# andres-quintela/manette

Hardware: AMD Instinct MI355X
Metric: env-steps/sec (ec x t_max frames per update) (higher is better)
Workload: dtype fp32

## Files before the change

### include/manette_hip.h

```cpp
#ifndef MANETTE_HIP_H
#define MANETTE_HIP_H

#include <stddef.h>
#include <stdint.h>

#ifdef __cplusplus
extern "C" {
#endif

typedef void *mt_stream_t;

enum {
  MT_OK = 0,
  MT_ERR_ARG = 1,
  MT_ERR_HIP = 2,
  MT_ERR_UNSUPPORTED = 3,
  MT_ERR_WORKSPACE = 4
};

enum { MT_ARCH_NIPS = 0, MT_ARCH_NATURE = 1, MT_ARCH_PWYX = 2, MT_ARCH_LSTM = 3, MT_ARCH_BAYESIAN = 4 };
enum { MT_ACT_RELU = 0, MT_ACT_LEAKY = 1 };
enum { MT_CLIP_IGNORE = 0, MT_CLIP_GLOBAL = 1 };

#define MT_NORM_PARTIALS 512
// ... 61 lines not shown
                            int E, int T, void *ws, size_t ws_bytes, const float *pi, const float *rep,
                            const float *v, const int32_t *a_idx, const int32_t *r_idx, const float *y,
                            const float *adv, float entropy_beta, float *grad, float *loss_terms,
                            float *norm_partials, mt_stream_t stream);

int mt_sample(const float *pi, const float *rep, int batch, int num_actions, int num_reps,
              uint64_t seed, int row0, uint64_t *counters, int32_t *a_idx, int32_t *r_idx, int32_t *pair,
              mt_stream_t stream);

enum { MT_POLICY_MULTINOMIAL = 0, MT_POLICY_EGREEDY = 1, MT_POLICY_ARGMAX = 2 };
typedef struct {
  int32_t mode;
  int32_t annealed;
  double epsilon;
  double annealing_steps;
  int64_t rows_per_call;
} mt_policy;

int mt_sample_policy(const mt_policy *policy, const float *pi, const float *rep, int batch, int num_actions,
                     int num_reps, uint64_t seed, int row0, uint64_t *counters, int32_t *a_idx, int32_t *r_idx,
                     int32_t *pair, mt_stream_t stream);
int mt_policy_draw_host(const mt_policy *policy, uint64_t seed, uint64_t global_row, uint64_t counter,
                        const float *pi, int num_actions, const float *rep, int num_reps, int32_t *a, int32_t *r);

int mt_returns(const float *rewards, const float *masks, const float *values, const float *v_boot,
               double gamma, int T, int E, float *y, float *adv, mt_stream_t stream);

int mt_loss_backward(const mt_net *net, const float *params, const uint8_t *obs, int batch,
                     void *ws, size_t ws_bytes, const float *pi, const float *rep, const float *v,
                     const int32_t *a_idx, const int32_t *r_idx, const float *y, const float *adv,
                     float entropy_beta, float *grad, float *loss_terms, mt_stream_t stream);

int mt_returns_loss_backward(const mt_net *net, const float *params, const uint8_t *obs, int T, int E, void *ws,
                             size_t ws_bytes, const float *pi, const float *rep, const float *values,
                             const int32_t *a_idx, const int32_t *r_idx, const float *rewards,
                             const float *masks, const float *v_boot, double gamma, float *y, float *adv,
                             float entropy_beta, float *grad, float *loss_terms, float *norm_partials,
                             mt_stream_t stream);
int mt_returns_loss_backward_boot(const mt_net *net, const float *params, const uint8_t *obs, int T, int E, void *ws,
                                  size_t ws_bytes, const float *pi, const float *rep, const float *values,
                                  const int32_t *a_idx, const int32_t *r_idx, const float *rewards,
                                  const float *masks, const void *boot_ws, size_t boot_ws_bytes, float *v_boot,
                                  double gamma, float *y, float *adv, float entropy_beta, float *grad,
                                  float *loss_terms, float *norm_partials, mt_stream_t stream);

int mt_grad_sumsq(const float *g, size_t n, float inv_scale, float *partials, mt_stream_t stream);
// ... 105 lines not shown
```

### manette_amd/_lib.py

```python
import ctypes as C
import os

HERE = os.path.dirname(os.path.abspath(__file__))
HIP_LIB = os.environ.get('MANETTE_HIP_LIB') or os.path.join(HERE, 'libmanette_hip.so')
HOST_LIB = os.path.join(HERE, 'libmanette_host.so')

MT_ARCH = {'NIPS': 0, 'NATURE': 1, 'PWYX': 2, 'LSTM': 3, 'BAYESIAN': 4}
MT_ACT = {'relu': 0, 'leaky_relu': 1}
MT_CLIP = {'ignore': 0, 'global': 1}
MT_NORM_PARTIALS = 512
MT_COMM_UID_BYTES = 128


class MTError(RuntimeError):
    pass


class mt_rollout_buffers(C.Structure):
    _fields_ = [(n, C.c_void_p) for n in ('states', 'values', 'idx', 'pi', 'rep', 'ws')] + \
               [('ws_bytes', C.c_size_t)] + \
               [(n, C.c_void_p) for n in ('counters', 'raw')] + [('src_rows', C.c_int32)] + \
               [(n, C.c_void_p) for n in ('pair', 'pair_host', 'meta', 'row_lut', 'col_lut', 'idx_host',
                                          'staging_host', 'meta_host', 'reward_host', 'over_host',
                                          'rm_host', 'frames_host', 'sync_host', 'train_ws')] + \
# ... 39 lines not shown
    'mt_net_create': (_I, [C.POINTER(mt_net_config), C.POINTER(_P)]),
    'mt_net_destroy': (None, [_P]),
    'mt_net_num_params': (_I, [_P, C.POINTER(_SZ)]),
    'mt_net_num_vars': (_I, [_P, C.POINTER(_I)]),
    'mt_net_var_info': (_I, [_P, _I, C.c_char_p, _I, C.POINTER(C.c_int64), C.POINTER(_I),
                             C.POINTER(_SZ), C.POINTER(_F)]),
    'mt_net_feature_dim': (_I, [_P, C.POINTER(_I)]),
    'mt_net_workspace_bytes': (_I, [_P, _I, C.POINTER(_SZ)]),
    'mt_net_workspace_region': (_I, [_P, _I, _I, _I, _I, _I, C.POINTER(_SZ), C.POINTER(_SZ)]),
    'mt_forward': (_I, [_P, _P, _P, _I, _P, _SZ, _P, _P, _P, _P]),
    'mt_lstm_frames_workspace_bytes': (_I, [_P, _I, _I, C.POINTER(_SZ)]),
    'mt_lstm_frames_forward': (_I, [_P, _P, _P, _I, _I, _I, _I, _P, _SZ, _P]),
    'mt_lstm_windows_forward': (_I, [_P, _P, _P, _I, _I, _I, _P, _SZ, _P, _P, _P, _P]),
    'mt_lstm_step_forward': (_I, [_P, _P, _P, _I, _I, _I, _P, _P, _P, _SZ, _P, _P, _P, _P]),
    'mt_lstm_frames_backward': (_I, [_P, _P, _P, _P, _I, _I, _P, _SZ, _P, _P, _P, _P, _P, _P, _P, _F, _P, _P, _P, _P]),
    'mt_forward_rows': (_I, [_P, _P, _P, _I, _P, _SZ, _P, _SZ, _I, _I, _P, _P, _P, _P]),
    'mt_forward_trunk': (_I, [_P, _P, _P, _I, _P, _SZ, _P]),
    'mt_forward_trunk_stacking': (_I, [_P, _P, _P, _P, _P, C.c_uint32, _P, _I, _P, _SZ, _P, _P]),
    'mt_forward_infer': (_I, [_P, _P, _P, _I, _P, _SZ, _P, _P, _P, _P]),
    'mt_sample': (_I, [_P, _P, _I, _I, _I, C.c_uint64, _I, _P, _P, _P, _P, _P]),
    'mt_sample_policy': (_I, [C.POINTER(mt_policy), _P, _P, _I, _I, _I, C.c_uint64, _I, _P, _P, _P, _P, _P]),
    'mt_policy_draw_host': (_I, [C.POINTER(mt_policy), C.c_uint64, C.c_uint64, C.c_uint64, _P, _I, _P, _I,
                                 C.POINTER(C.c_int32), C.POINTER(C.c_int32)]),
    'mt_rollout_set_policy': (_I, [_P, C.POINTER(mt_policy)]),
    'mt_returns': (_I, [_P, _P, _P, _P, C.c_double, _I, _I, _P, _P, _P]),
    'mt_loss_backward': (_I, [_P, _P, _P, _I, _P, _SZ, _P, _P, _P, _P, _P, _P, _P, _F, _P, _P, _P]),
    'mt_dropout_redraw': (_I, [_P, _P, _I, _P, _SZ, _P, _P, _P, _P]),
    'mt_dropout_mask_host': (_I, [C.c_uint64, C.c_uint64, C.c_uint64, _F, _P]),
    'mt_returns_loss_backward': (_I, [_P, _P, _P, _I, _I, _P, _SZ, _P, _P, _P, _P, _P, _P, _P, _P, C.c_double, _P, _P,
                                      _F, _P, _P, _P, _P]),
    'mt_returns_loss_backward_boot': (_I, [_P, _P, _P, _I, _I, _P, _SZ, _P, _P, _P, _P, _P, _P, _P, _P, _SZ, _P,
                                           C.c_double, _P, _P, _F, _P, _P, _P, _P]),
    'mt_grad_sumsq': (_I, [_P, _SZ, _F, _P, _P]),
    'mt_clip_rmsprop': (_I, [_P, _P, _P, _P, _SZ, _P, _P, _F, _F, _F, _F, _I, _F, _P, _P]),
    'mt_preprocess': (_I, [_P, _P, _P, _I, _I, _I, _P, _P, _P, _P, _P]),
    'mt_preprocess_pooled': (_I, [_P, _P, _P, _I, _I, _I, _P, _P, _P, _P, _P]),
    'mt_preprocess_resized': (_I, [_P, _P, _P, _I, _I, _P, _P, _P]),
    'mt_preprocess_frames': (_I, [_P, _P, _P, _I, _I, _P, _P, _P, _P, _P]),
    'mt_memory_push': (_I, [_P, _P, _P, _P, _I, _SZ, _P]),
    'mt_host_device_pointer': (_I, [_P, C.POINTER(_P)]),
    'mt_sum_slabs': (_I, [_P, _I, _SZ, _P, _P]),
    'mt_net_get_config': (_I, [_P, C.POINTER(mt_net_config)]),
    'mt_rollout_create': (_I, [_P, _I, _I, _P, _P, C.POINTER(mt_rollout_buffers), C.c_uint64, C.POINTER(_P)]),
    'mt_rollout_destroy': (None, [_P]),
    'mt_rollout_step': (_I, [_P, _P, _I, C.POINTER(C.c_int64), _P]),
    'mt_rollout_run': (_I, [_P, _P, C.POINTER(C.c_int64), _P]),
    'mt_rollout_stats': (_I, [_P, C.POINTER(C.c_double), _I]),
# ... 95 lines not shown
```

### manette_amd/build.py

```python
import os
import shutil
import subprocess
import sys

HERE = os.path.dirname(os.path.abspath(__file__))
CSRC = os.path.join(HERE, 'csrc')
HIP_SOURCES = ['net.hip', 'misc.hip', 'rollout.hip', 'comm.hip']
HIP_HEADERS = ['common.h', 'gemm.h', 'jobs.h', 'nips_bwd.h', 'trunk_fused.h', 'lstm.h', 'dconv.h', 'nature_bwd.h',
               'bayes.h']
HOST_SOURCES = ['runner.cpp', 'crc32c.cpp']
HIP_LIB = os.path.join(HERE, 'libmanette_hip.so')
PROBE_LIB = os.path.join(HERE, 'libmanette_hip_probe.so')
HOST_LIB = os.path.join(HERE, 'libmanette_host.so')
INCLUDE = os.path.join(os.path.dirname(HERE), 'include')


def _hipcc():
    for c in (os.environ.get('HIPCC'), '/opt/rocm/bin/hipcc', shutil.which('hipcc')):
        if c and os.path.exists(c):
            return c
    raise RuntimeError('hipcc not found')


def _stale(target, deps):
    if not os.path.exists(target):
        return True
    t = os.path.getmtime(target)
    return any(os.path.getmtime(d) > t for d in deps)


def build_hip(force=False, verbose=False, out=None, defines=()):
    target = out or HIP_LIB
# ... 60 lines not shown
```

### manette_amd/csrc/misc.hip

```cpp
#include <algorithm>
#include <atomic>
#include <cmath>

#include "common.h"

namespace mt {

static thread_local char g_err[512] = "";

void set_error(const char *fmt, ...) {
  va_list ap;
  va_start(ap, fmt);
  vsnprintf(g_err, sizeof(g_err), fmt, ap);
  va_end(ap);
}

__global__ void returns_kernel(const float *__restrict__ r, const float *__restrict__ mask,
                               const float *__restrict__ V, const float *__restrict__ VT,
                               double gamma, int T, int E, float *__restrict__ y,
                               float *__restrict__ adv) {
#pragma clang fp contract(off)
  const int e = blockIdx.x * blockDim.x + threadIdx.x;
  if (e >= E) return;
  const float g32 = __fmul_rn((float)gamma, VT[e]);
  double R = (double)r[(size_t)(T - 1) * E + e] + (double)g32 * (double)mask[(size_t)(T - 1) * E + e];
  y[(size_t)(T - 1) * E + e] = (float)R;
  adv[(size_t)(T - 1) * E + e] = (float)(R - (double)V[(size_t)(T - 1) * E + e]);
// ... 403 lines not shown
  MT_CHECK_ARG(pi && rep && counters && a_idx && r_idx, "null argument");
  MT_CHECK_ARG(batch >= 1 && num_actions >= 1 && num_reps >= 1 && row0 >= 0, "bad sizes");
  if (int rc = policy_check(policy, "mt_sample_policy")) return rc;
  hipLaunchKernelGGL(sample_kernel, dim3(cdiv(batch, 64)), dim3(64), 0, (hipStream_t)stream,
                     policy ? *policy : mt_policy{}, pi, rep, batch, num_actions, num_reps, seed, row0, counters,
                     a_idx, r_idx, pair);
  MT_LAUNCHED();
  return MT_OK;
}

extern "C" int mt_policy_draw_host(const mt_policy *policy, uint64_t seed, uint64_t global_row, uint64_t counter,
                                   const float *pi, int num_actions, const float *rep, int num_reps, int32_t *a,
                                   int32_t *r) {
  MT_CHECK_ARG(pi && rep && a && r, "null argument");
  MT_CHECK_ARG(num_actions >= 1 && num_reps >= 1, "bad sizes");
  if (int rc = policy_check(policy, "mt_policy_draw_host")) return rc;
  int ai, ri;
  policy_row(policy ? *policy : mt_policy{}, pi, num_actions, rep, num_reps, seed, global_row, counter, &ai, &ri);
  *a = ai;
  *r = ri;
  return MT_OK;
}

extern "C" int mt_graph_begin(mt_stream_t stream) {
  MT_CHECK_ARG(stream != nullptr, "graph capture needs a non-default stream");
  MT_HIP(hipStreamBeginCapture((hipStream_t)stream, hipStreamCaptureModeThreadLocal));
  return MT_OK;
}

extern "C" int mt_graph_end(mt_stream_t stream, void **graph_exec) {
  MT_CHECK_ARG(stream && graph_exec, "null argument");
  hipGraph_t g = nullptr;
  MT_HIP(hipStreamEndCapture((hipStream_t)stream, &g));
  hipGraphExec_t ex = nullptr;
  hipError_t e = hipGraphInstantiate(&ex, g, nullptr, nullptr, 0);
  (void)hipGraphDestroy(g);
  if (e != hipSuccess) {
    set_error("hipGraphInstantiate failed: %s", hipGetErrorString(e));
    return MT_ERR_HIP;
  }
  *graph_exec = (void *)ex;
  return MT_OK;
}

extern "C" int mt_graph_launch(void *graph_exec, mt_stream_t stream) {
  MT_CHECK_ARG(graph_exec, "null graph");
// ... 43 lines not shown
```

### manette_amd/csrc/nips_bwd.h

```cpp
#pragma once
#include "gemm.h"
#include "trunk_fused.h"

namespace mt {

struct NipsConvBwdJob {
  const uint8_t *X = nullptr;
  const float *act1 = nullptr, *dY2 = nullptr, *W2 = nullptr;
  float *dact1 = nullptr, *slab1 = nullptr, *slab2 = nullptr;
  int B = 0, act = 0;
  float alpha = 0.f;

  static constexpr int NT = 512;
  static constexpr int XROW = 24;
  static constexpr int XPLANE = 21 * XROW;
  static constexpr int X_BYTES = 64 * XPLANE;
  static constexpr int DS = 36;
  static constexpr int DY_FLOATS = 11 * 11 * DS;
  static constexpr int WS = 36;
  static constexpr int W2_FLOATS = 16 * 16 * WS;
  static constexpr int PS = 404;
  static constexpr int MAP_FLOATS = 16 * PS;
  static constexpr int SLAB1 = 257 * 16, SLAB2 = 257 * 32;
  static constexpr size_t LDS = X_BYTES + sizeof(float) * (DY_FLOATS + W2_FLOATS + 2 * MAP_FLOATS);
  static_assert(2 * sizeof(float) * (DY_FLOATS + MAP_FLOATS) <= LDS, "pair block stage");

  __host__ __device__ int pairs() const { return (B + 1) / 2; }
  __host__ __device__ int blocks() const { return B + pairs(); }

  struct DyAct {
    f32x4 yv[2], av[4];
  };
  __device__ __forceinline__ DyAct load_dy_act(int b) const {
    const int tid = threadIdx.x;
    const f32x4 *ys = reinterpret_cast<const f32x4 *>(dY2 + (size_t)b * 81 * 32);
    const f32x4 *as = reinterpret_cast<const f32x4 *>(act1 + (size_t)b * 400 * 16);
    DyAct d;
#pragma unroll
    for (int u = 0; u < 2; ++u) d.yv[u] = ys[min(tid + NT * u, 647)];
#pragma unroll
    for (int u = 0; u < 4; ++u) d.av[u] = as[min(tid + NT * u, 1599)];
    return d;
  }
  __device__ __forceinline__ void store_dy_act(const DyAct &d, float *dyp, float *a1t) const {
    const int tid = threadIdx.x;
    for (int i = tid; i < 121 * 8; i += NT) {
      const int p = i >> 3, Y = p / 11, Xc = p - 11 * Y;
// ... 10 lines not shown
    }
#pragma unroll
    for (int u = 0; u < 4; ++u) {
      const int i = tid + NT * u;
      if (i < 1600) {
        const int p = i >> 2, c = 4 * (i & 3);
#pragma unroll
        for (int e = 0; e < 4; ++e) a1t[(c + e) * PS + p] = d.av[u][e];
      }
    }
  }

  __device__ __forceinline__ void run(int bid, float *smem) const {
    if (bid < B)
      image_block(bid, smem);
    else
      pair_block(bid - B, smem);
  }

  __device__ __forceinline__ void image_block(int b, float *smem) const {
    float *dyp = smem;
    float *w2s = dyp + DY_FLOATS;
    float *a1t = w2s + W2_FLOATS;
    float *dat = a1t + MAP_FLOATS;
    uint8_t *xq = reinterpret_cast<uint8_t *>(dat + MAP_FLOATS);
    const int tid = threadIdx.x, lane = tid & 63, w = tid >> 6;
    const int r = lane & 15, g = lane >> 4;
    MT_PROBE_AT(3, b, 0);

    const uint4 *xs = reinterpret_cast<const uint4 *>(X + (size_t)b * 84 * 84 * 4);
    uint4 xv[4];
    {
      const int it = min(tid, 84 * 6 - 1), y = it / 6, jq = it - 6 * (it / 6);
#pragma unroll
      for (int v = 0; v < 4; ++v) xv[v] = xs[y * 21 + min(4 * jq + v, 20)];
    }
    const f32x4 *wsrc = reinterpret_cast<const f32x4 *>(W2);
    f32x4 wv[4];
#pragma unroll
    for (int u = 0; u < 4; ++u) wv[u] = wsrc[tid + NT * u];
    const DyAct da = load_dy_act(b);
    store_dy_act(da, dyp, a1t);
    if (tid < 84 * 6) {
      const int y = tid / 6, jq = tid - 6 * (tid / 6);
      uint8_t *row = xq + (y & 3) * 16 * XPLANE + (y >> 2) * XROW + 4 * jq;
#pragma unroll
      for (int p = 0; p < 4; ++p) {
        const uint32_t c0 = (&xv[0].x)[p], c1 = (&xv[1].x)[p], c2 = (&xv[2].x)[p], c3 = (&xv[3].x)[p];
// ... 28 lines not shown
#pragma unroll
        for (int t = 0; t < 4; ++t) af[t] = *reinterpret_cast<const f32x4 *>(dyp + off[t] - (a * 11 + bb) * DS + co0);
      };
      f32x4 acc[4];
#pragma unroll
      for (int t = 0; t < 4; ++t) acc[t] = f32x4{0.f, 0.f, 0.f, 0.f};
      f32x4 bf, af[4];
      frags(0, bf, af);
#pragma unroll
      for (int kc = 0; kc < 8; ++kc) {
        f32x4 bn, an[4];
        if (kc + 1 < 8) frags(kc + 1, bn, an);
#pragma unroll
        for (int s = 0; s < 4; ++s)
#pragma unroll
          for (int t = 0; t < 4; ++t)
            if (t < nt) acc[t] = __builtin_amdgcn_mfma_f32_16x16x4f32(af[t][s], bf[s], acc[t], 0, 0, 0);
        if (kc + 1 < 8) {
          bf = bn;
#pragma unroll
          for (int t = 0; t < 4; ++t) af[t] = an[t];
        }
      }
#pragma unroll
      for (int t = 0; t < 4; ++t)
#pragma unroll
        for (int i = 0; i < 4; ++i) {
          const int q = 16 * (t0 + t) + 4 * g + i;
          if (q < 100) {
            const int qy = q / 10, qx = q - 10 * qy;
            const int p = (2 * qy + py) * 20 + 2 * qx + px;
            const float v = acc[t][i] * act_bwd(a1t[r * PS + p], act, alpha);
            dat[r * PS + p] = v;
            if (dact1) dact1[((size_t)b * 400 + p) * 16 + r] = v;
          }
        }
    }
    __syncthreads();
    MT_PROBE_AT(3, b, 2);

    {
      f32x4 acc[2] = {f32x4{0.f, 0.f, 0.f, 0.f}, f32x4{0.f, 0.f, 0.f, 0.f}};
      float db = 0.f;
      const uint8_t *pl = xq + ((w & 3) * 16 + r) * XPLANE + (w >> 2) * XROW;
      auto frag = [&](int kc, f32x4 &bf, uint32_t &u0, uint32_t &u1) {
        const int p0 = 16 * kc + 4 * g, oy = p0 / 20, ox0 = p0 - 20 * oy;
        bf = *reinterpret_cast<const f32x4 *>(dat + r * PS + p0);
        const uint32_t *src = reinterpret_cast<const uint32_t *>(pl + oy * XROW + ox0);
        u0 = src[0];
        u1 = __builtin_amdgcn_alignbyte(src[1], src[0], 1);
      };
      f32x4 bf;
      uint32_t u0, u1;
      frag(0, bf, u0, u1);
#pragma unroll 5
      for (int kc = 0; kc < 25; ++kc) {
        f32x4 bn;
        uint32_t n0, n1;
        frag(min(kc + 1, 24), bn, n0, n1);
#pragma unroll
        for (int s = 0; s < 4; ++s) {
          acc[0] = __builtin_amdgcn_mfma_f32_16x16x4f32((float)((u0 >> (8 * s)) & 255u), bf[s], acc[0], 0, 0, 0);
          acc[1] = __builtin_amdgcn_mfma_f32_16x16x4f32((float)((u1 >> (8 * s)) & 255u), bf[s], acc[1], 0, 0, 0);
        }
        db += (bf[0] + bf[1]) + (bf[2] + bf[3]);
        bf = bn;
        u0 = n0;
        u1 = n1;
      }
      const float sc = 1.0f / 255.0f;
      float *o = slab1 + (size_t)b * SLAB1;
#pragma unroll
      for (int mt = 0; mt < 2; ++mt)
#pragma unroll
        for (int i = 0; i < 4; ++i) o[(16 * (2 * w + mt) + 4 * g + i) * 16 + r] = acc[mt][i] * sc;
      db += __shfl_xor(db, 16, 64);
      db += __shfl_xor(db, 32, 64);
      if (w == 0 && lane < 16) o[256 * 16 + r] = db;
    }
    MT_PROBE_AT(3, b, 4);
  }

  __device__ __forceinline__ void pair_block(int q, float *smem) const {
    const int lane = threadIdx.x & 63, w = threadIdx.x >> 6;
    const int r = lane & 15, g = lane >> 4;
    const int nimg = 2 * q + 1 < B ? 2 : 1;
    float *dyp[2] = {smem, smem + DY_FLOATS + MAP_FLOATS};
    float *a1t[2] = {smem + DY_FLOATS, smem + 2 * DY_FLOATS + MAP_FLOATS};
    MT_PROBE_AT(3, B + q, 0);
    const DyAct d0 = load_dy_act(2 * q), d1 = load_dy_act(min(2 * q + 1, B - 1));
    store_dy_act(d0, dyp[0], a1t[0]);
    if (nimg == 2) store_dy_act(d1, dyp[1], a1t[1]);
    __syncthreads();
    MT_PROBE_AT(3, B + q, 1);
    f32x4 acc[2][2];
#pragma unroll
    for (int mt = 0; mt < 2; ++mt) acc[mt][0] = acc[mt][1] = f32x4{0.f, 0.f, 0.f, 0.f};
    float db0 = 0.f, db1 = 0.f;
    const int ky = w >> 1, kx0 = 2 * (w & 1);
    for (int im = 0; im < nimg; ++im) {
      const float *dy = dyp[im], *at = a1t[im];
// ... 55 lines not shown
```

### manette_amd/csrc/trunk_fused.h

```cpp
#pragma once
#include "gemm.h"

#ifdef MT_PROBE
static __device__ unsigned long long mt_probe_buf[5 * 1024 * 8];
#define MT_PROBE_AT(k, b, p)                                                                     \
  do {                                                                                           \
    if (threadIdx.x == 0 && (b) < 1024) mt_probe_buf[((k) * 1024 + (b)) * 8 + (p)] = __builtin_amdgcn_s_memrealtime(); \
  } while (0)
#else
#define MT_PROBE_AT(k, b, p) \
  do {                       \
  } while (0)
#endif

namespace mt {

template <int C>
struct FusedNips {
  static constexpr int D = C / 4;
  static constexpr int ROWS2 = 9;
  static constexpr int ROWS1 = 4;
  static constexpr int RIN = 20;
  static constexpr int OW1 = 20, CO1 = 16, KK1 = 64 * C;
  static constexpr int OW2 = 9, CO2 = 32, KK2 = 256;
  static constexpr int A1S = 20;
  static constexpr int FEAT = OW2 * CO2;
  static constexpr int FLAT = ROWS2 * FEAT;
  static constexpr int F = 256;
  static constexpr int BPE = ROWS2;
  static constexpr int M1 = ROWS1 * OW1;
  static constexpr int MT1 = (M1 + 15) / 16;
  static constexpr int KC1 = KK1 / 16, KC2 = KK2 / 16;
  static constexpr int NW = C == 4 ? 8 : 4, NT = 64 * NW;
  static constexpr bool UNITS = C == 4;
  static constexpr int U1 = UNITS ? 2 * (MT1 - 1) + 4 : 0;
  static_assert(UNITS ? (C == 4 && KC1 == 16 && KC2 == 16 && MT1 == 5 && NW == 8)
                      : (KC1 % NW == 0 && KC2 % NW == 0), "K chunks split over the waves");
  static constexpr int IN_BYTES = RIN * 84 * C;
  static constexpr int FR_BYTES = RIN * 84 * D;
  static constexpr int RED_UNITS = (U1 > 8 ? U1 : 8) * 16 * CO1;
  static constexpr int RED_FLOATS = UNITS ? (RED_UNITS > FR_BYTES ? RED_UNITS : FR_BYTES)
                                          : NW * MT1 * 16 * CO1;
  static_assert(4 * FR_BYTES <= RED_FLOATS * 4, "staged frames alias the reduction buffer");
  static constexpr int W1P = KK1 + 4;
  static constexpr int W1T_FLOATS = UNITS ? CO1 * W1P : 0;
  static constexpr size_t LDS_BYTES = IN_BYTES + sizeof(float) * (RED_FLOATS + M1 * A1S + W1T_FLOATS);
  static constexpr int FC_BN = 16, FC_BM = 16, FC_KC = FEAT / 16;
  static constexpr int FC_SPLITS = 8;
};

template <int C, bool STACK>
__device__ __forceinline__ void nips_stage_rows(const uint8_t *__restrict__ obs, const StackSrc &st, int e, int i,
                                                uint8_t *xin, uint8_t *fr) {
  using Fz = FusedNips<C>;
  const size_t row0 = ((size_t)e * 84 + 8 * i) * 84 * C;
  if constexpr (!STACK) {
    const uint4 *src = reinterpret_cast<const uint4 *>(obs + row0);
    uint4 *dst = reinterpret_cast<uint4 *>(xin);
    for (int q = threadIdx.x; q < Fz::IN_BYTES / 16; q += Fz::NT) dst[q] = src[q];
    return;
  } else {
    __shared__ int s_p;
    const uint32_t tag = st.tag_base ? ((*st.tag_base + st.tag) & 0x1fffffffu) : st.tag;
    {
      const uint4 *src = reinterpret_cast<const uint4 *>(st.prev + row0);
      uint4 *dst = reinterpret_cast<uint4 *>(xin);
      for (int q = threadIdx.x; q < Fz::IN_BYTES / 16; q += Fz::NT) dst[q] = src[q];
    }
    int p;
    if (st.ready) {
      if (threadIdx.x == 0) s_p = wait_published(st.ready, e, tag, st.status);
      MT_PROBE_AT(0, blockIdx.x, 5);
      __syncthreads();
      p = min(max(s_p, 0), 4);
      const size_t F = (size_t)84 * 84 * Fz::D, lo = 4 * e * F, hi = lo + 4 * F;
      for (int q = threadIdx.x; q < p * (Fz::FR_BYTES / 16); q += Fz::NT) {
        const int j = q / (Fz::FR_BYTES / 16), qq = q - j * (Fz::FR_BYTES / 16);
        const size_t off = (((size_t)4 * e + j) * 84 + 8 * i) * 84 * Fz::D + 16 * (size_t)qq;
        reinterpret_cast<uint4 *>(fr + j * Fz::FR_BYTES)[qq] = ld_published16(st.frames, off, lo, hi);
      }
      __syncthreads();
    } else {
      if (threadIdx.x == 0) s_p = st.count ? st.count[e] : 0;
      if (st.count) {
        const size_t f0 = ((size_t)4 * e * 84 + 8 * i) * 84 * Fz::D;
        const uint4 *fs = reinterpret_cast<const uint4 *>(st.frames + f0);
        for (int q = threadIdx.x; q < Fz::FR_BYTES / 16; q += Fz::NT) reinterpret_cast<uint4 *>(fr)[q] = fs[q];
      }
      __syncthreads();
      p = st.count ? min(max(s_p, 1), 4) : 0;
      if (p > 1) {
        for (int q = threadIdx.x; q < (p - 1) * (Fz::FR_BYTES / 16); q += Fz::NT) {
          const int j = 1 + q / (Fz::FR_BYTES / 16), qq = q - (j - 1) * (Fz::FR_BYTES / 16);
          const size_t fj = (((size_t)4 * e + j) * 84 + 8 * i) * 84 * Fz::D;
          reinterpret_cast<uint4 *>(fr + j * Fz::FR_BYTES)[qq] = reinterpret_cast<const uint4 *>(st.frames + fj)[qq];
        }
        __syncthreads();
      }
    }
    uint32_t *xw = reinterpret_cast<uint32_t *>(xin);
    uint32_t *ow = reinterpret_cast<uint32_t *>(st.out + row0);
    const int own = (i == Fz::ROWS2 - 1 ? Fz::RIN : 8) * 84 * Fz::D;
    for (int w = threadIdx.x; w < Fz::RIN * 84 * Fz::D; w += Fz::NT) {
      uint32_t v = p < 4 ? xw[w] >> (8 * p) : 0u;
      for (int j = 0; j < p; ++j) v |= (uint32_t)fr[j * Fz::FR_BYTES + w] << (8 * (4 - p + j));
      xw[w] = v;
      if (w < own) ow[w] = v;
    }
  }
}

template <int C, int NCH>
__device__ __forceinline__ f32x4 nips_conv1_unit(const uint8_t *xin, const float *w1t, int t, int c0, int r, int g) {
  using Fz = FusedNips<C>;
  f32x4 acc0 = f32x4{0.f, 0.f, 0.f, 0.f}, acc1 = acc0;
  const float sc = 1.0f / 255.0f;
  const int m = min(t * 16 + r, Fz::M1 - 1);
  const int orow = m / Fz::OW1, ox = m - orow * Fz::OW1;
  const uint8_t *xb = xin + ((4 * orow) * 84 + 4 * ox) * C;
  uint32_t au[NCH];
  f32x4 bw[NCH];
#pragma unroll
  for (int j = 0; j < NCH; ++j) {
    const int kpos = 4 * (c0 + j) + g;
    au[j] = *reinterpret_cast<const uint32_t *>(xb + ((kpos >> 3) * 84 + (kpos & 7)) * C);
    bw[j] = *reinterpret_cast<const f32x4 *>(w1t + r * Fz::W1P + 16 * (c0 + j) + 4 * g);
  }
  __builtin_amdgcn_sched_barrier(0);
#pragma unroll
  for (int j = 0; j < NCH; ++j) {
    const uint32_t u = au[j];
    const f32x4 a = f32x4{(float)(u & 0xff) * sc, (float)((u >> 8) & 0xff) * sc, (float)((u >> 16) & 0xff) * sc,
                          (float)(u >> 24) * sc};
#pragma unroll
    for (int s = 0; s < 4; ++s) {
      if (j & 1)
        acc1 = __builtin_amdgcn_mfma_f32_16x16x4f32(a[s], bw[j][s], acc1, 0, 0, 0);
      else
        acc0 = __builtin_amdgcn_mfma_f32_16x16x4f32(a[s], bw[j][s], acc0, 0, 0, 0);
    }
  }
  return acc0 + acc1;
}

template <int C, bool STACK>
__global__ __launch_bounds__(FusedNips<C>::NT) void nips_conv_kernel(const uint8_t *__restrict__ obs, StackSrc st, int B,
                                                        const float *__restrict__ W1, const float *__restrict__ W2,
                                                        int act, float alpha, float *__restrict__ act2,
                                                        float *__restrict__ act1) {
  using Fz = FusedNips<C>;
  extern __shared__ __attribute__((aligned(16))) float smem[];
  float *red = smem;
  float *a1 = red + Fz::RED_FLOATS;
  float *w1t = a1 + Fz::M1 * Fz::A1S;
  uint8_t *xin = reinterpret_cast<uint8_t *>(w1t + Fz::W1T_FLOATS);
  uint8_t *fr = reinterpret_cast<uint8_t *>(red);

  const int nb = gridDim.x;
  const int bid = blockIdx.x;
  MT_PROBE_AT(0, bid, 0);
  const int L = (nb % 8 == 0) ? (bid % 8) * (nb / 8) + bid / 8 : bid;
  const int e = L / Fz::BPE, i = L - e * Fz::BPE;
  const int lane = threadIdx.x & 63, w = threadIdx.x >> 6;
  const int r = lane & 15, g = lane >> 4;

  constexpr int NW = Fz::NW;
  constexpr int J1 = Fz::UNITS ? 1 : Fz::KC1 / NW;
  float b1f[J1][4];
  if constexpr (Fz::UNITS) {
    constexpr int NQ = Fz::KK1 * Fz::CO1 / 4;
    f32x4 wv[(NQ + Fz::NT - 1) / Fz::NT];
#pragma unroll
    for (int u = 0; u < (NQ + Fz::NT - 1) / Fz::NT; ++u)
      wv[u] = reinterpret_cast<const f32x4 *>(W1)[min((int)threadIdx.x + Fz::NT * u, NQ - 1)];
#pragma unroll
    for (int u = 0; u < (NQ + Fz::NT - 1) / Fz::NT; ++u) {
      const int q = threadIdx.x + Fz::NT * u;
      if (q < NQ) {
        const int k = q >> 2, c4 = (q & 3) * 4;
#pragma unroll
        for (int e2 = 0; e2 < 4; ++e2) w1t[(c4 + e2) * Fz::W1P + k] = wv[u][e2];
      }
    }
  } else {
#pragma unroll
    for (int j = 0; j < J1; ++j) {
      const int k0 = 16 * (w + NW * j) + 4 * g;
#pragma unroll
      for (int s = 0; s < 4; ++s) b1f[j][s] = W1[(size_t)(k0 + s) * Fz::CO1 + r];
    }
  }
  nips_stage_rows<C, STACK>(obs, st, e, i, xin, fr);
  __syncthreads();
  MT_PROBE_AT(0, bid, 1);

  if constexpr (Fz::UNITS) {
    const int wu = __builtin_amdgcn_readfirstlane(w);
    const f32x4 acc = nips_conv1_unit<C, 8>(xin, w1t, wu >> 1, 8 * (wu & 1), r, g);
    f32x4 acc4 = f32x4{0.f, 0.f, 0.f, 0.f};
    if (wu < 4) acc4 = nips_conv1_unit<C, 4>(xin, w1t, 4, 4 * wu, r, g);
    MT_PROBE_AT(0, bid, 6);
#pragma unroll
    for (int q = 0; q < 4; ++q) red[(w * 16 + g * 4 + q) * Fz::CO1 + r] = acc[q];
    if (wu < 4)
#pragma unroll
      for (int q = 0; q < 4; ++q) red[((8 + w) * 16 + g * 4 + q) * Fz::CO1 + r] = acc4[q];
  } else   {
    f32x4 acc[Fz::MT1];
#pragma unroll
    for (int t = 0; t < Fz::MT1; ++t) acc[t] = f32x4{0.f, 0.f, 0.f, 0.f};
    const float sc = 1.0f / 255.0f;
#pragma unroll
    for (int j = 0; j < J1; ++j) {
      const int k0 = 16 * (w + NW * j) + 4 * g;
      const int kpos = k0 / C, ci = k0 - kpos * C;
      const int ky = kpos >> 3, kx = kpos & 7;
      f32x4 a[Fz::MT1];
#pragma unroll
      for (int t = 0; t < Fz::MT1; ++t) {
        const int m = min(t * 16 + r, Fz::M1 - 1);
        const int orow = m / Fz::OW1, ox = m - orow * Fz::OW1;
        const uint32_t u = *reinterpret_cast<const uint32_t *>(xin + ((4 * orow + ky) * 84 + 4 * ox + kx) * C + ci);
        a[t] = f32x4{(float)(u & 0xff) * sc, (float)((u >> 8) & 0xff) * sc, (float)((u >> 16) & 0xff) * sc,
                     (float)(u >> 24) * sc};
      }
#pragma unroll
      for (int s = 0; s < 4; ++s)
#pragma unroll
        for (int t = 0; t < Fz::MT1; ++t) acc[t] = __builtin_amdgcn_mfma_f32_16x16x4f32(a[t][s], b1f[j][s], acc[t], 0, 0, 0);
    }
    MT_PROBE_AT(0, bid, 6);
#pragma unroll
    for (int t = 0; t < Fz::MT1; ++t)
#pragma unroll
      for (int q = 0; q < 4; ++q) red[(w * Fz::MT1 * 16 + t * 16 + g * 4 + q) * Fz::CO1 + r] = acc[t][q];
  }
  constexpr int J2 = Fz::UNITS ? 4 : Fz::KC2 / NW;
  constexpr int NT2 = Fz::UNITS ? 1 : 2;
  float b2f[J2][NT2][4];
#pragma unroll
  for (int j = 0; j < J2; ++j) {
    const int k0 = 16 * (Fz::UNITS ? 4 * ((w >> 1) & 3) + j : w + NW * j) + 4 * g;
#pragma unroll
    for (int nt = 0; nt < NT2; ++nt)
#pragma unroll
      for (int s = 0; s < 4; ++s)
        b2f[j][nt][s] = W2[(size_t)(k0 + s) * Fz::CO2 + (Fz::UNITS ? (w & 1) : nt) * 16 + r];
  }
  __syncthreads();
  MT_PROBE_AT(0, bid, 7);
  {
    const float *b1 = W1 + (size_t)Fz::KK1 * Fz::CO1;
    constexpr int P = Fz::MT1 * 16 * Fz::CO1;
    for (int idx = threadIdx.x; idx < Fz::M1 * Fz::CO1; idx += Fz::NT) {
      const int m = idx / Fz::CO1, n = idx - m * Fz::CO1;
      float s;
      if constexpr (Fz::UNITS) {
        const int t = m >> 4, rr = m & 15;
        if (t < 4)
          s = red[((2 * t) * 16 + rr) * Fz::CO1 + n] + red[((2 * t + 1) * 16 + rr) * Fz::CO1 + n];
        else
          s = ((red[(8 * 16 + rr) * Fz::CO1 + n] + red[(9 * 16 + rr) * Fz::CO1 + n]) + red[(10 * 16 + rr) * Fz::CO1 + n]) +
              red[(11 * 16 + rr) * Fz::CO1 + n];
      } else {
        s = red[idx];
#pragma unroll
        for (int v = 1; v < NW; ++v) s += red[v * P + idx];
      }
      const float y = act_fwd(s + b1[n], act, alpha);
      a1[m * Fz::A1S + n] = y;
      const int orow = m / Fz::OW1, cx = m - orow * Fz::OW1;
      if (act1 && (orow < 2 || i == Fz::ROWS2 - 1))
        act1[(((size_t)e * Fz::OW1 + 2 * i + orow) * Fz::OW1 + cx) * Fz::CO1 + n] = y;
    }
  }
  __syncthreads();
  MT_PROBE_AT(0, bid, 2);

  if constexpr (Fz::UNITS) {
    if (w < 8) {
      const int kq = w >> 1;
      f32x4 acc0 = f32x4{0.f, 0.f, 0.f, 0.f}, acc1 = acc0;
      const int ox = min(r, Fz::OW2 - 1);
#pragma unroll
      for (int j = 0; j < J2; ++j) {
        const f32x4 a = *reinterpret_cast<const f32x4 *>(a1 + (kq * Fz::OW1 + 2 * ox + j) * Fz::A1S + 4 * g);
#pragma unroll
        for (int s = 0; s < 4; ++s) {
          if (j & 1)
            acc1 = __builtin_amdgcn_mfma_f32_16x16x4f32(a[s], b2f[j][0][s], acc1, 0, 0, 0);
          else
            acc0 = __builtin_amdgcn_mfma_f32_16x16x4f32(a[s], b2f[j][0][s], acc0, 0, 0, 0);
        }
      }
      const f32x4 acc = acc0 + acc1;
#pragma unroll
      for (int q = 0; q < 4; ++q) red[(w * 16 + g * 4 + q) * 16 + r] = acc[q];
    }
  } else   {
// ... 325 lines not shown
```

Measured before the change: 765,300.

## Use split-bf16 MFMA for NIPS conv1 forward and weight-gradient

Replaces the fp32 16x16x4 MFMA loops in the fused NIPS conv1 forward and in the conv1 weight-gradient backward with bf16 MFMAs. Byte inputs are exactly representable in bf16, and the fp32 operands (weights, dact) are split into three bf16 parts (hi/mid/lo) so the result stays close to fp32. The forward path also drops the cross-wave LDS reduction and an extra barrier, because each wave now covers the full K for one tile and applies bias and activation directly. In exchange it runs three MFMAs per operand pair, uses more LDS for the bf16 staging buffers, and gives slightly different rounding.

```diff
diff --git a/include/manette_hip.h b/include/manette_hip.h
--- a/include/manette_hip.h
+++ b/include/manette_hip.h
@@ -107,6 +107,8 @@
                      int32_t *pair, mt_stream_t stream);
 int mt_policy_draw_host(const mt_policy *policy, uint64_t seed, uint64_t global_row, uint64_t counter,
                         const float *pi, int num_actions, const float *rep, int num_reps, int32_t *a, int32_t *r);
+
+int mt_split3_bf16_host(const float *x, size_t n, uint16_t *parts, uint16_t *bytes);
 
 int mt_returns(const float *rewards, const float *masks, const float *values, const float *v_boot,
                double gamma, int T, int E, float *y, float *adv, mt_stream_t stream);
diff --git a/manette_amd/_lib.py b/manette_amd/_lib.py
--- a/manette_amd/_lib.py
+++ b/manette_amd/_lib.py
@@ -85,7 +85,8 @@
     'mt_sample_policy': (_I, [C.POINTER(mt_policy), _P, _P, _I, _I, _I, C.c_uint64, _I, _P, _P, _P, _P, _P]),
     'mt_policy_draw_host': (_I, [C.POINTER(mt_policy), C.c_uint64, C.c_uint64, C.c_uint64, _P, _I, _P, _I,
                                  C.POINTER(C.c_int32), C.POINTER(C.c_int32)]),
-    'mt_rollout_set_policy': (_I, [_P, C.POINTER(mt_policy)]),
+    'mt_split3_bf16_host': (_I, [_P, _SZ, _P, _P]),
+    'mt_rollout_set_policy':(_I, [_P, C.POINTER(mt_policy)]),
     'mt_returns': (_I, [_P, _P, _P, _P, C.c_double, _I, _I, _P, _P, _P]),
     'mt_loss_backward': (_I, [_P, _P, _P, _I, _P, _SZ, _P, _P, _P, _P, _P, _P, _P, _F, _P, _P, _P]),
     'mt_dropout_redraw': (_I, [_P, _P, _I, _P, _SZ, _P, _P, _P, _P]),
diff --git a/manette_amd/build.py b/manette_amd/build.py
--- a/manette_amd/build.py
+++ b/manette_amd/build.py
@@ -7,7 +7,7 @@
 CSRC = os.path.join(HERE, 'csrc')
 HIP_SOURCES = ['net.hip', 'misc.hip', 'rollout.hip', 'comm.hip']
 HIP_HEADERS = ['common.h', 'gemm.h', 'jobs.h', 'nips_bwd.h', 'trunk_fused.h', 'lstm.h', 'dconv.h', 'nature_bwd.h',
-               'bayes.h']
+               'bayes.h', 'split_bf16.h']
 HOST_SOURCES = ['runner.cpp', 'crc32c.cpp']
 HIP_LIB = os.path.join(HERE, 'libmanette_hip.so')
 PROBE_LIB = os.path.join(HERE, 'libmanette_hip_probe.so')
diff --git a/manette_amd/csrc/misc.hip b/manette_amd/csrc/misc.hip
--- a/manette_amd/csrc/misc.hip
+++ b/manette_amd/csrc/misc.hip
@@ -3,6 +3,7 @@
 #include <cmath>
 
 #include "common.h"
+#include "split_bf16.h"
 
 namespace mt {
 
@@ -452,6 +453,19 @@
   return MT_OK;
 }
 
+extern "C" int mt_split3_bf16_host(const float *x, size_t n, uint16_t *parts, uint16_t *bytes) {
+  MT_CHECK_ARG((x && parts) || n == 0, "null argument");
+  for (size_t i = 0; i < n; ++i) {
+    const Bf16x3 s = split3_bf16(x[i]);
+    parts[3 * i] = s.hi;
+    parts[3 * i + 1] = s.mid;
+    parts[3 * i + 2] = s.lo;
+  }
+  if (bytes)
+    for (uint32_t b = 0; b < 256; ++b) bytes[b] = bf16_from_byte(b);
+  return MT_OK;
+}
+
 extern "C" int mt_graph_begin(mt_stream_t stream) {
   MT_CHECK_ARG(stream != nullptr, "graph capture needs a non-default stream");
   MT_HIP(hipStreamBeginCapture((hipStream_t)stream, hipStreamCaptureModeThreadLocal));
diff --git a/manette_amd/csrc/nips_bwd.h b/manette_amd/csrc/nips_bwd.h
--- a/manette_amd/csrc/nips_bwd.h
+++ b/manette_amd/csrc/nips_bwd.h
@@ -21,8 +21,11 @@
   static constexpr int W2_FLOATS = 16 * 16 * WS;
   static constexpr int PS = 404;
   static constexpr int MAP_FLOATS = 16 * PS;
+  static constexpr int PSB = 400;
+  static constexpr int DATB_BYTES = 3 * 16 * PSB * 2;
+  static constexpr int DB_FLOATS = 8 * 16;
   static constexpr int SLAB1 = 257 * 16, SLAB2 = 257 * 32;
-  static constexpr size_t LDS = X_BYTES + sizeof(float) * (DY_FLOATS + W2_FLOATS + 2 * MAP_FLOATS);
+  static constexpr size_t LDS = X_BYTES + sizeof(float) * (DY_FLOATS + W2_FLOATS + MAP_FLOATS + DB_FLOATS) + DATB_BYTES;
   static_assert(2 * sizeof(float) * (DY_FLOATS + MAP_FLOATS) <= LDS, "pair block stage");
 
   __host__ __device__ int pairs() const { return (B + 1) / 2; }
@@ -79,8 +82,9 @@
     float *dyp = smem;
     float *w2s = dyp + DY_FLOATS;
     float *a1t = w2s + W2_FLOATS;
-    float *dat = a1t + MAP_FLOATS;
-    uint8_t *xq = reinterpret_cast<uint8_t *>(dat + MAP_FLOATS);
+    float *dbs = a1t + MAP_FLOATS;
+    uint16_t *datb = reinterpret_cast<uint16_t *>(dbs + DB_FLOATS);
+    uint8_t *xq = reinterpret_cast<uint8_t *>(datb) + DATB_BYTES;
     const int tid = threadIdx.x, lane = tid & 63, w = tid >> 6;
     const int r = lane & 15, g = lane >> 4;
     MT_PROBE_AT(3, b, 0);
@@ -155,6 +159,7 @@
           for (int t = 0; t < 4; ++t) af[t] = an[t];
         }
       }
+      float db = 0.f;
 #pragma unroll
       for (int t = 0; t < 4; ++t)
 #pragma unroll
@@ -164,52 +169,74 @@
             const int qy = q / 10, qx = q - 10 * qy;
             const int p = (2 * qy + py) * 20 + 2 * qx + px;
             const float v = acc[t][i] * act_bwd(a1t[r * PS + p], act, alpha);
-            dat[r * PS + p] = v;
+            const Bf16x3 s = split3_bf16(v);
+            datb[r * PSB + p] = s.hi;
+            datb[(16 + r) * PSB + p] = s.mid;
+            datb[(32 + r) * PSB + p] = s.lo;
+            db += v;
             if (dact1) dact1[((size_t)b * 400 + p) * 16 + r] = v;
           }
         }
+      db += __shfl_xor(db, 16, 64);
+      db += __shfl_xor(db, 32, 64);
+      if (lane < 16) dbs[w * 16 + r] = db;
     }
     __syncthreads();
     MT_PROBE_AT(3, b, 2);
 
     {
-      f32x4 acc[2] = {f32x4{0.f, 0.f, 0.f, 0.f}, f32x4{0.f, 0.f, 0.f, 0.f}};
-      float db = 0.f;
+      typedef short s16x4 __attribute__((ext_vector_type(4)));
+      f32x4 acc[2][3];
+#pragma unroll
+      for (int mt = 0; mt < 2; ++mt)
+#pragma unroll
+        for (int pn = 0; pn < 3; ++pn) acc[mt][pn] = f32x4{0.f, 0.f, 0.f, 0.f};
       const uint8_t *pl = xq + ((w & 3) * 16 + r) * XPLANE + (w >> 2) * XROW;
-      auto frag = [&](int kc, f32x4 &bf, uint32_t &u0, uint32_t &u1) {
+      auto frag = [&](int kc, uint2 (&bf)[3], uint32_t &u0, uint32_t &u1) {
         const int p0 = 16 * kc + 4 * g, oy = p0 / 20, ox0 = p0 - 20 * oy;
-        bf = *reinterpret_cast<const f32x4 *>(dat + r * PS + p0);
+#pragma unroll
+        for (int pn = 0; pn < 3; ++pn) bf[pn] = *reinterpret_cast<const uint2 *>(datb + (pn * 16 + r) * PSB + p0);
         const uint32_t *src = reinterpret_cast<const uint32_t *>(pl + oy * XROW + ox0);
         u0 = src[0];
         u1 = __builtin_amdgcn_alignbyte(src[1], src[0], 1);
       };
-      f32x4 bf;
+      auto bytes_bf16 = [](uint32_t u) {
+        return __builtin_bit_cast(s16x4, make_uint2(bf16x2_from_bytes(u & 255u, (u >> 8) & 255u),
+                                                    bf16x2_from_bytes((u >> 16) & 255u, u >> 24)));
+      };
+      uint2 bf[3];
       uint32_t u0, u1;
       frag(0, bf, u0, u1);
 #pragma unroll 5
       for (int kc = 0; kc < 25; ++kc) {
-        f32x4 bn;
+        uint2 bn[3];
         uint32_t n0, n1;
         frag(min(kc + 1, 24), bn, n0, n1);
-#pragma unroll
-        for (int s = 0; s < 4; ++s) {
-          acc[0] = __builtin_amdgcn_mfma_f32_16x16x4f32((float)((u0 >> (8 * s)) & 255u), bf[s], acc[0], 0, 0, 0);
-          acc[1] = __builtin_amdgcn_mfma_f32_16x16x4f32((float)((u1 >> (8 * s)) & 255u), bf[s], acc[1], 0, 0, 0);
+        const s16x4 a0 = bytes_bf16(u0), a1 = bytes_bf16(u1);
+#pragma unroll
+        for (int pn = 0; pn < 3; ++pn) {
+          const s16x4 bv = __builtin_bit_cast(s16x4, bf[pn]);
+          acc[0][pn] = __builtin_amdgcn_mfma_f32_16x16x16bf16_1k(a0, bv, acc[0][pn], 0, 0, 0);
+          acc[1][pn] = __builtin_amdgcn_mfma_f32_16x16x16bf16_1k(a1, bv, acc[1][pn], 0, 0, 0);
+          bf[pn] = bn[pn];
         }
-        db += (bf[0] + bf[1]) + (bf[2] + bf[3]);
-        bf = bn;
         u0 = n0;
         u1 = n1;
       }
       const float sc = 1.0f / 255.0f;
       float *o = slab1 + (size_t)b * SLAB1;
 #pragma unroll
-      for (int mt = 0; mt < 2; ++mt)
-#pragma unroll
-        for (int i = 0; i < 4; ++i) o[(16 * (2 * w + mt) + 4 * g + i) * 16 + r] = acc[mt][i] * sc;
-      db += __shfl_xor(db, 16, 64);
-      db += __shfl_xor(db, 32, 64);
-      if (w == 0 && lane < 16) o[256 * 16 + r] = db;
+      for (int mt = 0; mt < 2; ++mt) {
+        const f32x4 s = (acc[mt][2] + acc[mt][1]) + acc[mt][0];
+#pragma unroll
+        for (int i = 0; i < 4; ++i) o[(16 * (2 * w + mt) + 4 * g + i) * 16 + r] = s[i] * sc;
+      }
+      if (w == 0 && lane < 16) {
+        float db = dbs[r];
+#pragma unroll
+        for (int v = 1; v < 8; ++v) db += dbs[v * 16 + r];
+        o[256 * 16 + r] = db;
+      }
     }
     MT_PROBE_AT(3, b, 4);
   }
diff --git a/manette_amd/csrc/split_bf16.h b/manette_amd/csrc/split_bf16.h
--- /dev/null
+++ b/manette_amd/csrc/split_bf16.h
@@ -0,0 +1,31 @@
+#pragma once
+#include <cstdint>
+
+namespace mt {
+
+__host__ __device__ __forceinline__ uint32_t f32_bits(float x) { return __builtin_bit_cast(uint32_t, x); }
+__host__ __device__ __forceinline__ float bf16_to_f32(uint16_t h) { return __builtin_bit_cast(float, (uint32_t)h << 16); }
+__host__ __device__ __forceinline__ uint16_t bf16_rn(float x) {
+  const uint32_t u = f32_bits(x);
+  return (uint16_t)((u + 0x7fffu + ((u >> 16) & 1u)) >> 16);
+}
+
+struct Bf16x3 {
+  uint16_t hi, mid, lo;
+};
+__host__ __device__ __forceinline__ Bf16x3 split3_bf16(float x) {
+  Bf16x3 s;
+  s.hi = bf16_rn(x);
+  const float r1 = x - bf16_to_f32(s.hi);
+  s.mid = bf16_rn(r1);
+  const float r2 = r1 - bf16_to_f32(s.mid);
+  s.lo = bf16_rn(r2);
+  return s;
+}
+
+__host__ __device__ __forceinline__ uint16_t bf16_from_byte(uint32_t b) { return (uint16_t)(f32_bits((float)b) >> 16); }
+__host__ __device__ __forceinline__ uint32_t bf16x2_from_bytes(uint32_t b0, uint32_t b1) {
+  return (f32_bits((float)b0) >> 16) | (f32_bits((float)b1) & 0xffff0000u);
+}
+
+}
diff --git a/manette_amd/csrc/trunk_fused.h b/manette_amd/csrc/trunk_fused.h
--- a/manette_amd/csrc/trunk_fused.h
+++ b/manette_amd/csrc/trunk_fused.h
@@ -1,5 +1,6 @@
 #pragma once
 #include "gemm.h"
+#include "split_bf16.h"
 
 #ifdef MT_PROBE
 static __device__ unsigned long long mt_probe_buf[5 * 1024 * 8];
@@ -33,31 +34,45 @@
   static constexpr int KC1 = KK1 / 16, KC2 = KK2 / 16;
   static constexpr int NW = C == 4 ? 8 : 4, NT = 64 * NW;
   static constexpr bool UNITS = C == 4;
-  static constexpr int U1 = UNITS ? 2 * (MT1 - 1) + 4 : 0;
-  static_assert(UNITS ? (C == 4 && KC1 == 16 && KC2 == 16 && MT1 == 5 && NW == 8)
+  static_assert(UNITS ? (C == 4 && KK1 == 256 && KC2 == 16 && MT1 == 5 && M1 == 16 * MT1 && NW == 8)
                       : (KC1 % NW == 0 && KC2 % NW == 0), "K chunks split over the waves");
   static constexpr int IN_BYTES = RIN * 84 * C;
   static constexpr int FR_BYTES = RIN * 84 * D;
-  static constexpr int RED_UNITS = (U1 > 8 ? U1 : 8) * 16 * CO1;
-  static constexpr int RED_FLOATS = UNITS ? (RED_UNITS > FR_BYTES ? RED_UNITS : FR_BYTES)
+  static constexpr int RED_FLOATS = UNITS ? 8 * 16 * 16
                                           : NW * MT1 * 16 * CO1;
   static_assert(4 * FR_BYTES <= RED_FLOATS * 4, "staged frames alias the reduction buffer");
-  static constexpr int W1P = KK1 + 4;
-  static constexpr int W1T_FLOATS = UNITS ? CO1 * W1P : 0;
-  static constexpr size_t LDS_BYTES = IN_BYTES + sizeof(float) * (RED_FLOATS + M1 * A1S + W1T_FLOATS);
+  static constexpr int W1P = KK1 + 8;
+  static constexpr int W1B_BYTES = UNITS ? 3 * CO1 * W1P * 2 : 0;
+  static constexpr int XB_BYTES = UNITS ? 2 * IN_BYTES : 0;
+  static constexpr size_t LDS_BYTES = IN_BYTES + sizeof(float) * (RED_FLOATS + M1 * A1S) + W1B_BYTES + XB_BYTES;
   static constexpr int FC_BN = 16, FC_BM = 16, FC_KC = FEAT / 16;
   static constexpr int FC_SPLITS = 8;
 };
 
+__device__ __forceinline__ uint2 bf16x4_from_u8x4(uint32_t u) {
+  return make_uint2(bf16x2_from_bytes(u & 0xff, (u >> 8) & 0xff), bf16x2_from_bytes((u >> 16) & 0xff, u >> 24));
+}
+
 template <int C, bool STACK>
 __device__ __forceinline__ void nips_stage_rows(const uint8_t *__restrict__ obs, const StackSrc &st, int e, int i,
-                                                uint8_t *xin, uint8_t *fr) {
+                                                uint8_t *xin, uint8_t *fr, uint16_t *xb) {
   using Fz = FusedNips<C>;
   const size_t row0 = ((size_t)e * 84 + 8 * i) * 84 * C;
   if constexpr (!STACK) {
     const uint4 *src = reinterpret_cast<const uint4 *>(obs + row0);
-    uint4 *dst = reinterpret_cast<uint4 *>(xin);
-    for (int q = threadIdx.x; q < Fz::IN_BYTES / 16; q += Fz::NT) dst[q] = src[q];
+    if constexpr (Fz::UNITS) {
+      uint4 *dst = reinterpret_cast<uint4 *>(xb);
+      for (int q = threadIdx.x; q < Fz::IN_BYTES / 16; q += Fz::NT) {
+        const uint4 v = src[q];
+        const uint2 a = bf16x4_from_u8x4(v.x), b = bf16x4_from_u8x4(v.y), c = bf16x4_from_u8x4(v.z),
+                    d = bf16x4_from_u8x4(v.w);
+        dst[2 * q] = make_uint4(a.x, a.y, b.x, b.y);
+        dst[2 * q + 1] = make_uint4(c.x, c.y, d.x, d.y);
+      }
+    } else {
+      uint4 *dst = reinterpret_cast<uint4 *>(xin);
+      for (int q = threadIdx.x; q < Fz::IN_BYTES / 16; q += Fz::NT) dst[q] = src[q];
+    }
     return;
   } else {
     __shared__ int s_p;
@@ -104,43 +119,37 @@
     for (int w = threadIdx.x; w < Fz::RIN * 84 * Fz::D; w += Fz::NT) {
       uint32_t v = p < 4 ? xw[w] >> (8 * p) : 0u;
       for (int j = 0; j < p; ++j) v |= (uint32_t)fr[j * Fz::FR_BYTES + w] << (8 * (4 - p + j));
-      xw[w] = v;
+      if constexpr (Fz::UNITS)
+        reinterpret_cast<uint2 *>(xb)[w] = bf16x4_from_u8x4(v);
+      else
+        xw[w] = v;
       if (w < own) ow[w] = v;
     }
   }
 }
 
-template <int C, int NCH>
-__device__ __forceinline__ f32x4 nips_conv1_unit(const uint8_t *xin, const float *w1t, int t, int c0, int r, int g) {
+typedef __bf16 bf16x8 __attribute__((ext_vector_type(8)));
+template <int C>
+__device__ __forceinline__ f32x4 nips_conv1_tile_bf16(const uint16_t *xb, const uint16_t *w1b, int t, int r, int g) {
   using Fz = FusedNips<C>;
-  f32x4 acc0 = f32x4{0.f, 0.f, 0.f, 0.f}, acc1 = acc0;
-  const float sc = 1.0f / 255.0f;
-  const int m = min(t * 16 + r, Fz::M1 - 1);
+  static_assert(C == 4, "8 k of a lane = 2 pixels x 4 channels");
+  const int m = t * 16 + r;
   const int orow = m / Fz::OW1, ox = m - orow * Fz::OW1;
-  const uint8_t *xb = xin + ((4 * orow) * 84 + 4 * ox) * C;
-  uint32_t au[NCH];
-  f32x4 bw[NCH];
-#pragma unroll
-  for (int j = 0; j < NCH; ++j) {
-    const int kpos = 4 * (c0 + j) + g;
-    au[j] = *reinterpret_cast<const uint32_t *>(xb + ((kpos >> 3) * 84 + (kpos & 7)) * C);
-    bw[j] = *reinterpret_cast<const f32x4 *>(w1t + r * Fz::W1P + 16 * (c0 + j) + 4 * g);
-  }
-  __builtin_amdgcn_sched_barrier(0);
-#pragma unroll
-  for (int j = 0; j < NCH; ++j) {
-    const uint32_t u = au[j];
-    const f32x4 a = f32x4{(float)(u & 0xff) * sc, (float)((u >> 8) & 0xff) * sc, (float)((u >> 16) & 0xff) * sc,
-                          (float)(u >> 24) * sc};
-#pragma unroll
-    for (int s = 0; s < 4; ++s) {
-      if (j & 1)
-        acc1 = __builtin_amdgcn_mfma_f32_16x16x4f32(a[s], bw[j][s], acc1, 0, 0, 0);
-      else
-        acc0 = __builtin_amdgcn_mfma_f32_16x16x4f32(a[s], bw[j][s], acc0, 0, 0, 0);
-    }
-  }
-  return acc0 + acc1;
+  const uint16_t *xa = xb + ((4 * orow) * 84 + 4 * ox + 2 * g) * C;
+  const uint16_t *wb = w1b + r * Fz::W1P + 8 * g;
+  f32x4 acc[3];
+#pragma unroll
+  for (int p = 0; p < 3; ++p) acc[p] = f32x4{0.f, 0.f, 0.f, 0.f};
+#pragma unroll
+  for (int ky = 0; ky < 8; ++ky) {
+    const bf16x8 a = *reinterpret_cast<const bf16x8 *>(xa + ky * 84 * C);
+#pragma unroll
+    for (int p = 0; p < 3; ++p) {
+      const bf16x8 b = *reinterpret_cast<const bf16x8 *>(wb + p * Fz::CO1 * Fz::W1P + 32 * ky);
+      acc[p] = __builtin_amdgcn_mfma_f32_16x16x32_bf16(a, b, acc[p], 0, 0, 0);
+    }
+  }
+  return (acc[2] + acc[1]) + acc[0];
 }
 
 template <int C, bool STACK>
@@ -152,8 +161,9 @@
   extern __shared__ __attribute__((aligned(16))) float smem[];
   float *red = smem;
   float *a1 = red + Fz::RED_FLOATS;
-  float *w1t = a1 + Fz::M1 * Fz::A1S;
-  uint8_t *xin = reinterpret_cast<uint8_t *>(w1t + Fz::W1T_FLOATS);
+  uint16_t *w1b = reinterpret_cast<uint16_t *>(a1 + Fz::M1 * Fz::A1S);
+  uint16_t *xb = w1b + Fz::W1B_BYTES / 2;
+  uint8_t *xin = reinterpret_cast<uint8_t *>(xb + Fz::XB_BYTES / 2);
   uint8_t *fr = reinterpret_cast<uint8_t *>(red);
 
   const int nb = gridDim.x;
@@ -168,19 +178,18 @@
   constexpr int J1 = Fz::UNITS ? 1 : Fz::KC1 / NW;
   float b1f[J1][4];
   if constexpr (Fz::UNITS) {
-    constexpr int NQ = Fz::KK1 * Fz::CO1 / 4;
-    f32x4 wv[(NQ + Fz::NT - 1) / Fz::NT];
-#pragma unroll
-    for (int u = 0; u < (NQ + Fz::NT - 1) / Fz::NT; ++u)
-      wv[u] = reinterpret_cast<const f32x4 *>(W1)[min((int)threadIdx.x + Fz::NT * u, NQ - 1)];
-#pragma unroll
-    for (int u = 0; u < (NQ + Fz::NT - 1) / Fz::NT; ++u) {
-      const int q = threadIdx.x + Fz::NT * u;
-      if (q < NQ) {
-        const int k = q >> 2, c4 = (q & 3) * 4;
-#pragma unroll
-        for (int e2 = 0; e2 < 4; ++e2) w1t[(c4 + e2) * Fz::W1P + k] = wv[u][e2];
-      }
+    static_assert(Fz::KK1 / 2 * (Fz::CO1 / 4) == Fz::NT, "one (k pair, channel quad) per thread");
+    const int kp = threadIdx.x >> 2, c4 = (threadIdx.x & 3) * 4;
+    const f32x4 wa = reinterpret_cast<const f32x4 *>(W1)[(2 * kp) * (Fz::CO1 / 4) + (threadIdx.x & 3)];
+    const f32x4 wb = reinterpret_cast<const f32x4 *>(W1)[(2 * kp + 1) * (Fz::CO1 / 4) + (threadIdx.x & 3)];
+    uint32_t *w1w = reinterpret_cast<uint32_t *>(w1b);
+#pragma unroll
+    for (int e2 = 0; e2 < 4; ++e2) {
+      const Bf16x3 sa = split3_bf16(wa[e2]), sb = split3_bf16(wb[e2]);
+      uint32_t *dst = w1w + (c4 + e2) * (Fz::W1P / 2) + kp;
+      dst[0] = sa.hi | ((uint32_t)sb.hi << 16);
+      dst[Fz::CO1 * Fz::W1P / 2] = sa.mid | ((uint32_t)sb.mid << 16);
+      dst[2 * Fz::CO1 * Fz::W1P / 2] = sa.lo | ((uint32_t)sb.lo << 16);
     }
   } else {
 #pragma unroll
@@ -190,21 +199,43 @@
       for (int s = 0; s < 4; ++s) b1f[j][s] = W1[(size_t)(k0 + s) * Fz::CO1 + r];
     }
   }
-  nips_stage_rows<C, STACK>(obs, st, e, i, xin, fr);
+  nips_stage_rows<C, STACK>(obs, st, e, i, xin, fr, xb);
   __syncthreads();
   MT_PROBE_AT(0, bid, 1);
 
+  constexpr int J2 = Fz::UNITS ? 4 : Fz::KC2 / NW;
+  constexpr int NT2 = Fz::UNITS ? 1 : 2;
+  float b2f[J2][NT2][4];
+  auto load_b2f = [&]() {
+#pragma unroll
+    for (int j = 0; j < J2; ++j) {
+      const int k0 = 16 * (Fz::UNITS ? 4 * ((w >> 1) & 3) + j : w + NW * j) + 4 * g;
+#pragma unroll
+      for (int nt = 0; nt < NT2; ++nt)
+#pragma unroll
+        for (int s = 0; s < 4; ++s)
+          b2f[j][nt][s] = W2[(size_t)(k0 + s) * Fz::CO2 + (Fz::UNITS ? (w & 1) : nt) * 16 + r];
+    }
+  };
+
   if constexpr (Fz::UNITS) {
+    load_b2f();
     const int wu = __builtin_amdgcn_readfirstlane(w);
-    const f32x4 acc = nips_conv1_unit<C, 8>(xin, w1t, wu >> 1, 8 * (wu & 1), r, g);
-    f32x4 acc4 = f32x4{0.f, 0.f, 0.f, 0.f};
-    if (wu < 4) acc4 = nips_conv1_unit<C, 4>(xin, w1t, 4, 4 * wu, r, g);
-    MT_PROBE_AT(0, bid, 6);
-#pragma unroll
-    for (int q = 0; q < 4; ++q) red[(w * 16 + g * 4 + q) * Fz::CO1 + r] = acc[q];
-    if (wu < 4)
-#pragma unroll
-      for (int q = 0; q < 4; ++q) red[((8 + w) * 16 + g * 4 + q) * Fz::CO1 + r] = acc4[q];
+    if (wu < Fz::MT1) {
+      const float bias = W1[(size_t)Fz::KK1 * Fz::CO1 + r];
+      const f32x4 acc = nips_conv1_tile_bf16<C>(xb, w1b, wu, r, g);
+      MT_PROBE_AT(0, bid, 6);
+      const float sc = 1.0f / 255.0f;
+#pragma unroll
+      for (int q = 0; q < 4; ++q) {
+        const int m = wu * 16 + g * 4 + q;
+        const float y = act_fwd(acc[q] * sc + bias, act, alpha);
+        a1[m * Fz::A1S + r] = y;
+        const int orow = m / Fz::OW1, cx = m - orow * Fz::OW1;
+        if (act1 && (orow < 2 || i == Fz::ROWS2 - 1))
+          act1[(((size_t)e * Fz::OW1 + 2 * i + orow) * Fz::OW1 + cx) * Fz::CO1 + r] = y;
+      }
+    }
   } else   {
     f32x4 acc[Fz::MT1];
 #pragma unroll
@@ -235,46 +266,25 @@
 #pragma unroll
       for (int q = 0; q < 4; ++q) red[(w * Fz::MT1 * 16 + t * 16 + g * 4 + q) * Fz::CO1 + r] = acc[t][q];
   }
-  constexpr int J2 = Fz::UNITS ? 4 : Fz::KC2 / NW;
-  constexpr int NT2 = Fz::UNITS ? 1 : 2;
-  float b2f[J2][NT2][4];
-#pragma unroll
-  for (int j = 0; j < J2; ++j) {
-    const int k0 = 16 * (Fz::UNITS ? 4 * ((w >> 1) & 3) + j : w + NW * j) + 4 * g;
-#pragma unroll
-    for (int nt = 0; nt < NT2; ++nt)
-#pragma unroll
-      for (int s = 0; s < 4; ++s)
-        b2f[j][nt][s] = W2[(size_t)(k0 + s) * Fz::CO2 + (Fz::UNITS ? (w & 1) : nt) * 16 + r];
-  }
+  if constexpr (!Fz::UNITS) load_b2f();
   __syncthreads();
   MT_PROBE_AT(0, bid, 7);
-  {
+  if constexpr (!Fz::UNITS) {
     const float *b1 = W1 + (size_t)Fz::KK1 * Fz::CO1;
     constexpr int P = Fz::MT1 * 16 * Fz::CO1;
     for (int idx = threadIdx.x; idx < Fz::M1 * Fz::CO1; idx += Fz::NT) {
       const int m = idx / Fz::CO1, n = idx - m * Fz::CO1;
-      float s;
-      if constexpr (Fz::UNITS) {
-        const int t = m >> 4, rr = m & 15;
-        if (t < 4)
-          s = red[((2 * t) * 16 + rr) * Fz::CO1 + n] + red[((2 * t + 1) * 16 + rr) * Fz::CO1 + n];
-        else
-          s = ((red[(8 * 16 + rr) * Fz::CO1 + n] + red[(9 * 16 + rr) * Fz::CO1 + n]) + red[(10 * 16 + rr) * Fz::CO1 + n]) +
-              red[(11 * 16 + rr) * Fz::CO1 + n];
-      } else {
-        s = red[idx];
-#pragma unroll
-        for (int v = 1; v < NW; ++v) s += red[v * P + idx];
-      }
+      float s = red[idx];
+#pragma unroll
+      for (int v = 1; v < NW; ++v) s += red[v * P + idx];
       const float y = act_fwd(s + b1[n], act, alpha);
       a1[m * Fz::A1S + n] = y;
       const int orow = m / Fz::OW1, cx = m - orow * Fz::OW1;
       if (act1 && (orow < 2 || i == Fz::ROWS2 - 1))
         act1[(((size_t)e * Fz::OW1 + 2 * i + orow) * Fz::OW1 + cx) * Fz::CO1 + n] = y;
     }
-  }
-  __syncthreads();
+    __syncthreads();
+  }
   MT_PROBE_AT(0, bid, 2);
 
   if constexpr (Fz::UNITS) {
```

Result: faster. 817,600, median of 6 (+6.8%).
